# noce2/FluidFramework

Hardware: AMD Instinct MI355X
Metric: sequenced merge-tree ops applied/sec (node) at 100k docs; bit-exact text+props (higher is better)
Workload: dtype int32; 1 GPU; c3: 100000 docs/GPU x 10000 sequenced ops, 8 writers, refSeq lag <= 64, insert 0.5 / remove 0.3 / annotate 0.2; docs_total=100000, docs_per_gpu=100000, ops_per_doc=10000, parallelism=doc-shard x1

## Files before the change

fluidframework_amd/csrc/mt_engine.h:

```cpp
#pragma once
#include <type_traits>

#include "mt_device.h"

#define LDS_AS __attribute__((address_space(3)))
#define GLB_AS __attribute__((address_space(1)))

template <bool kLogT> struct TierLdsT {
    static constexpr bool kLds = true;
    static constexpr bool kLog = kLogT;
    static constexpr bool kPaged = false;
    static constexpr bool kLive = false;
    static constexpr int kOvlBits = 32;
    static constexpr bool kMayGrow = false;
    static constexpr bool kOvf = false;
    typedef uint32_t O_v;
    typedef LDS_AS v4i *A_t;
    typedef LDS_AS uint32_t *O_t;
    typedef LDS_AS v4u *B_t;
    typedef LDS_AS v2i *H_t;
};
template <bool kLogT> struct TierGlbT {
    static constexpr bool kLds = false;
    static constexpr bool kLog = kLogT;
// ... 1980 lines not shown
        const int kept = scour_range(d, bstart, b, 1);
        if (d.status) return;
        wsync<T>();
        if (lane() == 0) d.flg[b] = 0;
        wsync<T>();
        if (kept < old && kept < MT_HALF && d.depth > 1)
            pack(d, 0, b);
        else if (kept < old && ordon(d))
            ord_canon(d, 0, b);
    }
}

TD bool lds_room(DocT<T> &d, const mt_op_rec &op) {
    if (d.n + 3 > d.S_cap) return false;
    if (d.depth + 2 > MT_LV) return false;
    const int nb0 = nbr(d, 0);
    int need_heap = op.kind == MT_OP_INSERT ? 1 : nb0 + 3;
    if (d.heap_n + need_heap > d.H_cap) return false;
    bool ok = true;
    for (int l = 0; l < d.depth; l++) ok = ok && nbr(d, l) + 3 + 24 <= bcap(d, l);
    if (op.kind == MT_OP_REMOVE && oslot_short(d, op_cli(op))) ok = false;
    return ok;
}

TD int live_room(DocT<T> &d, const mt_op_rec &op) {
    if (d.n + 3 > d.S_cap) return 1;
    for (int l = 0; l < d.depth; l++)
        if (nbr(d, l) + 3 + 24 > bcap(d, l)) return 2;
    const int nb0 = nbr(d, 0);
    if (d.heap_n + (op.kind == MT_OP_INSERT ? 1 : nb0 + 3) > d.H_cap) return 3;
    const int nt = op.kind == MT_OP_INSERT && !(op.flags & MT_F_MARKER) ? max(op.pos2, 0) : 0;
    const int tslack = max(d.T_cap / 8, 4096);
    if (d.text_top + nt + tslack > d.T_cap) {
        text_gc(d);
        if (d.text_top + nt + tslack > d.T_cap) return 4;
    }
    const int span = op.kind == MT_OP_ANNOTATE ? min(max(op.pos2 - op.pos1, 0), d.n) + 2 : 0;
    const int np = span + (op.props != MT_NO_PROPS ? 1 : 0) + MT_WAVE;
    if (d.props_top + np > d.P_cap) {
        props_gc(d);
        if (d.props_top + np > d.P_cap) return 5;
    }
    if ((op.flags & MT_F_LOCAL) && d.g_n + 1 > d.LG) return 12;
    return 0;
}

struct OpIn {
    mt_op_rec op;
    u64 pay_lo, pay_hi;
    bool pay_ok;
    bool nl;
    bool pay_lane = false;
    uint32_t pay_v = 0;
};

__device__ __forceinline__ uint16_t pay_unit(const OpIn &in, int j) {
    const u64 w = j < 4 ? (in.pay_lo >> (16 * j)) : (in.pay_hi >> (16 * (j - 4)));
    return (uint16_t)(w & 0xFFFF);
}

TD int first_v0(DocT<T> &d, int from) {
    for (int base = from; base < d.n; base += MT_WAVE) {
        const int i = base + lane();
        const bool v = i < d.n;
        v4i a;
        u64 o;
        load_ao(d, i, v, a, o);
        const u64 m = ballot(v && obs_len(a) > 0);
        if (m) return base + first_lane(m);
    }
    return -1;
}

#ifdef MT_PROF
TD void op_insert_impl(DocT<T> &d, const OpIn &in, const GLB_AS uint16_t *tin, const GLB_AS uint32_t *pin);
TD void op_insert(DocT<T> &d, const OpIn &in, const GLB_AS uint16_t *tin, const GLB_AS uint32_t *pin) {
    PROF_WRAP_BEGIN
    op_insert_impl(d, in, tin, pin);
    PROF_WRAP_END(6)
    
}
TD void op_insert_impl(DocT<T> &d, const OpIn &in, const GLB_AS uint16_t *tin, const GLB_AS uint32_t *pin) {
#else
TD void op_insert(DocT<T> &d, const OpIn &in, const GLB_AS uint16_t *tin, const GLB_AS uint32_t *pin) {
#endif
    const mt_op_rec &op = in.op;
    const int r = op.ref_seq, c = op_cli(op), seq = op.seq, p = op.pos1;
    const bool quiet = (op.flags & MT_F_LOAD) != 0;
    const bool marker = (op.flags & MT_F_MARKER) != 0;
    const int slen = marker ? 1 : op.pos2;
    if (slen > 0 && !marker && !text_ensure(d, slen)) return;
    if (slen > 0 && op.props != MT_NO_PROPS && !props_ensure(d, 1)) return;
    P2_T0(13)
    int carry = 0, split_i = -1, split_q = 0, ip = -1, js = -1;
    for (int base = 0; base < d.n; base += MT_WAVE) {
        const int i = base + lane();
        const bool v = i < d.n;
        v4i a;
        u64 o;
        load_ao(d, i, v, a, o);
        const int vl = v ? vlen(d, a, o, r, c) : 0;
        const int inc = wave_scan_incl(vl);
        const int pex = carry + inc - vl, pin_ = carry + inc;
        const u64 ms = ballot(v && pex < p && p < pin_);
        if (ms) {
            const int l = first_lane(ms);
            split_i = base + l;
// ... 16 lines not shown
        if (ballot(v && pex > p)) break;
    }
    P2_T1(13)
    if (split_i >= 0) {
        split_seg(d, split_i, split_q);
        if (d.status) return;
        ip = js = split_i + 1;
    } else if (ip < 0 && carry == p) {
        ip = d.n;
    }
    Cb cb;
    if (!quiet) cb = cb_begin(d, (T::kLive && d.lop) ? -1 : seq, MT_OP_INSERT);
    if (slen == 0) {
        if (quiet) return;
        cb.n = 1;
        cb_log(d, -1);
        cb_log(d, 0);
        if constexpr (T::kLog) {
            if (d.rich && cb_room(d, 2 + (op.props != MT_NO_PROPS ? 2 * (int)(pin[op.props] & 0xFFFF) : 0))) {
                int np = -1;
                if (op.props != MT_NO_PROPS) {
                    const GLB_AS uint32_t *rec = pin + op.props;
                    np = 0;
                    for (uint32_t j = 0; j < (rec[0] & 0xFFFF); j++) {
                        if (rec[2 + 2 * j] == MT_VAL_NULL) continue;
                        if (lane() == 0) {
                            d.dlog[d.dlog_n + 2 + 2 * np] = (int32_t)rec[1 + 2 * j];
                            d.dlog[d.dlog_n + 3 + 2 * np] = (int32_t)rec[2 + 2 * j];
                        }
                        np++;
                    }
                }
                if (lane() == 0) {
                    d.dlog[d.dlog_n] = (np >= 0 ? 2 : 0) | (ordon(d) ? 4 : 0);
                    d.dlog[d.dlog_n + 1] = np;
                }
                d.dlog_n += 2 + 2 * max(np, 0);
                cb_log_ext(d, 0u, 0, -1, false);
            }
        }
        cb.h = fnv_u64(cb.h, fnv_u32(fnv_u32(MT_FNV_OFF, (uint32_t)-1), 0u));
        cb_end(d, cb);
        return;
    }
    if (ip < 0) {
        fail(d, MT_DOC_INSERT_FAILED);
        return;
    }
    if (d.n + 1 > d.S_cap) {
        fail_cap(d, 1);
        return;
    }
    uint32_t ph = 0, nomatch = 0;
    if (op.props != MT_NO_PROPS) {
        ph = (uint32_t)d.props_top;
        d.props_top++;
        const GLB_AS uint32_t *rec = pin + op.props;
        const uint32_t cntk = rec[0] & 0xFFFF;
        int cn = 0;
        for (uint32_t j = 0; j < cntk; j++) cn += rec[2 + 2 * j] != MT_VAL_NULL;
        if (cn > MT_KMAX) {
            fail(d, MT_DOC_CAPACITY);
            return;
        }
        if (lane() == 0) {
            GLB_AS uint32_t *t = prec(d, d.props_half, ph);
            uint32_t n = 0;
            for (uint32_t j = 0; j < cntk; j++) {
                if (rec[2 + 2 * j] == MT_VAL_NULL) continue;
                t[1 + 2 * n] = rec[1 + 2 * j];
                t[2 + 2 * n] = rec[2 + 2 * j];
                n++;
            }
            t[0] = n;
        }
#ifndef MT_NO_Q4
        bool nm = false;
        for (uint32_t j = 0; j < cntk; j++) {
            const uint32_t v = rec[2 + 2 * j];
            nm = nm || (v != MT_VAL_NULL && (v & MT_VAL_NOMATCH_BIT));
        }
        if (nm) nomatch = SEGF_NOMATCH;
#endif
#ifndef MT_NO_PSIG
        uint32_t sig = 0;
        for (uint32_t j = 0; j < cntk; j++) {
            const uint32_t v = rec[2 + 2 * j];
            if (v != MT_VAL_NULL) sig += mt_psig_mix(rec[1 + 2 * j], v);
        }
        nomatch = psig_put(nomatch, sig);
#endif
    }
    int bstart;
    int B = blk_find(d, 0, ip, false, bstart);
    if (B < 0) {
        FAIL_INTERNAL(d);
        return;
    }
    int bend = bstart + cntr(d, 0, B);
    int x = (js >= 0 && js < bend) ? js : bend;
    if constexpr (T::kLive) {
        while (!d.lop && x == bend) {
            const int s0 = first_v0(d, bend);
            if (s0 < 0 || !is_local_seq(uni(d.A[s0].y)) || B + 1 >= nbr(d, 0)) break;
            B++;
            bstart = bend;
            bend += cntr(d, 0, B);
            x = (js >= 0 && js < bend) ? js : bend;
        }
    }
    uint32_t toff, segw = 0;
    if (marker) {
        toff = op.payload;
    } else {
        toff = (uint32_t)d.text_top;
        GLB_AS uint16_t *dst = text_base(d, d.text_half) + d.text_top;
        bool anynl = false, lastnl = false;
        if (in.pay_ok) {
            const uint16_t u = lane() < slen ? (in.pay_lane ? (uint16_t)in.pay_v : pay_unit(in, lane())) : (uint16_t)0;
            if (lane() < slen) dst[lane()] = u;
            anynl = ballot(lane() < slen && u == (uint16_t)'\n') != 0ull;
            lastnl = ballot(lane() == slen - 1 && u == (uint16_t)'\n') != 0ull;
        } else {
            for (int j = lane(); j < slen; j += MT_WAVE) {
                const uint16_t u = tin[op.payload + j];
                dst[j] = u;
                anynl = anynl || u == (uint16_t)'\n';
                lastnl = lastnl || (j == slen - 1 && u == (uint16_t)'\n');
            }
            anynl = ballot(anynl) != 0ull;
            lastnl = ballot(lastnl) != 0ull;
        }
#ifdef MT_NO_NONL
        anynl = true;
#endif
        d.text_top += slen;
        segw = SEGF_NL_KNOWN | (lastnl ? SEGF_NL : 0u) | (anynl ? 0u : SEGF_NONL);
    }
    P2_T0(15)
    seg_move_right(d, x, 1);
    P2_T1(15)
    mark_dirty(d, x);
    const uint32_t uid = (uint32_t)d.next_uid;
    if (lane() == 0) {
        d.A[x] = v4i{slen, seq, MT_RSEQ_NONE, pack_cli(c, 0)};
// ... 159 lines not shown
            npd++;
        }
        uint32_t nv = v;
#ifndef MT_NO_Q4
        if (comb == MT_COMBINE_TABLE) {
            const GLB_AS uint32_t *tab = rec + 1 + 2 * cntk;
            nv = tab[1];
            if (!absent) {
                const uint32_t old = t[2 + 2 * idx];
                bool hit = false;
                for (uint32_t q = 0; q < tab[0]; q++)
                    if (tab[2 + 2 * q] == old) {
                        nv = tab[3 + 2 * q];
                        hit = true;
                    }
                if (!hit) return false;
            }
        }
#endif
#ifndef MT_NO_PSIG
        if (idx >= 0) sg -= mt_psig_mix(k, t[2 + 2 * idx]);
        if (nv != MT_VAL_NULL) sg += mt_psig_mix(k, nv);
#endif
        if (nv == MT_VAL_NULL) {
            if (idx >= 0) {
                for (uint32_t q = (uint32_t)idx + 1; q < n; q++) {
                    t[2 * q - 1] = t[2 * q + 1];
                    t[2 * q] = t[2 * q + 2];
                }
                n--;
            }
        } else if (idx >= 0) {
            t[2 + 2 * idx] = nv;
        } else {
            if (n >= MT_KMAX) return false;
            t[1 + 2 * n] = k;
            t[2 + 2 * n] = nv;
            n++;
        }
    }
    t[0] = n;
#ifndef MT_NO_PSIG
    if (psig) *psig = sg;
#endif
    sh = fnv_u32(sh, (uint32_t)npd);
    if (nomatch && *nomatch) {
        bool nm = false;
        for (uint32_t q = 0; q < n; q++) nm = nm || (t[2 + 2 * q] & MT_VAL_NOMATCH_BIT) != 0;
        *nomatch = nm;
    }
    return true;
}

TD bool range_mark(DocT<T> &d, const mt_op_rec &op, const GLB_AS uint32_t *rec, int &carry, int &ocarry,
                   Cb &cb) {
    const int r = op.ref_seq, c = op_cli(op), seq = op.seq, p1 = op.pos1, p2 = op.pos2;
    const bool rem = op.kind == MT_OP_REMOVE;
    compute_ends(d);
    if (!rem) gsync_rd();
    int last_b = -1;
    const int L = lane();
    const int nblk = nbr(d, 0);
    bool rec_nm = false;
#ifndef MT_NO_Q4
    if (!rem) {
        rec_nm = (rec[0] >> 16) == MT_COMBINE_TABLE;
        for (uint32_t j = 0; j < (rec[0] & 0xFFFFu); j++) {
            const uint32_t v = rec[2 + 2 * j];
            rec_nm = rec_nm || (v != MT_VAL_NULL && (v & MT_VAL_NOMATCH_BIT));
        }
    }
#endif
    for (int base = 0; base < d.n; base += MT_WAVE) {
        if (!rem && !props_ensure(d, MT_WAVE)) return true;
        const int i = base + L;
        const bool v = i < d.n;
        v4i a;
        u64 o;
        load_ao(d, i, v, a, o);
        const v4u bv = d.Bv[v ? i : 0];
        const int vl = v ? vlen(d, a, o, r, c) : 0;
        const int inc = wave_scan_incl(vl);
        const int pex = carry + inc - vl, pin_ = carry + inc;
        const bool sel = v && vl > 0 && pex < p2 && pin_ > p1;
        const u64 sel_m = ballot(sel);
        if (sel_m) mark_dirty(d, base + first_lane(sel_m));
        bool newly = false, bad = false, spill = false, want_ovf = false;
        bool lrem = false;
        if constexpr (T::kLive) lrem = rem && sel && !d.lop && is_local_seq(a.z);
        const bool ovl_any = rem && ballot(sel && a.z != MT_RSEQ_NONE && !lrem);
        if (ovl_any) {
            if (d.ocs == 0) d.ocs = oslot_take(d, c);
            if (d.ocs > 32) d.wide = 1;
            if (d.ocs && lane() == 0) d.oslot[2 * (d.ocs - 1) + 1] = seq;
        }
        if (rem && sel) {
            if (lrem) {
                a.z = seq;
                a.w = pack_cli(seg_cli(a), c);
                d.A[i] = a;
            } else if (a.z != MT_RSEQ_NONE) {
                bool ovf = false;
                if constexpr (T::kPaged && T::kOvf) ovf = d.ocs == 0 || (o & MT_OVF_BIT);
                if (ovf) {
                    want_ovf = true;
                } else if (d.ocs == 0) {
                    if (T::kOvlBits < 64)
                        spill = true;
                    else
                        bad = true;
                } else {
                    d.O[i] = (typename T::O_v)(o | (1ull << (d.ocs - 1)));
                }
            } else {
                newly = true;
                a.z = seq;
                a.w = pack_cli(seg_cli(a), c);
                d.A[i] = a;
                if constexpr (T::kLive) {
                    if (d.lop) {
                        PendQ pq = pq_get(d, i);
                        if (pq_push(pq, d.lg))
                            pq_put(d, i, pq);
                        else
                            bad = true;
                    }
                }
            }
        }
        if constexpr (T::kPaged && T::kOvf) {
            if (ballot(want_ovf) && !ovf_mark(d, want_ovf, i, o, c, seq)) bad = true;
        }
        uint32_t nh = 0;
        if (!rem && sel) nh = (uint32_t)(d.props_top + __popcll(sel_m & ((1ull << L) - 1ull)));
        const int ol = v ? obs_len(a) : 0;
        const int oinc = wave_scan_incl(ol);
        const int opos = ocarry + oinc - ol;
        const bool entry = rem ? newly : sel;
        u64 sh = fnv_u32(fnv_u32(MT_FNV_OFF, (uint32_t)opos), (uint32_t)a.x);
        if (!rem && sel) {
            int unused = 0;
            bool nm = rec_nm || (bv.w & SEGF_NOMATCH) != 0;
            PendQ pw = pq_zero();
            if constexpr (T::kLive) {
                PendQ pq = pq_get(d, i);
                if (d.lop) {
                    if (pq_push(pq, d.lg))
                        pq_put(d, i, pq);
                    else
                        bad = true;
                } else {
                    pw = pq;
                }
            }
            uint32_t sg = psig_of(bv.w);
            if (!annotate_record(d, bv.y, nh, rec, sh, (GLB_AS int32_t *)nullptr, unused, &nm, pw, nullptr, &sg))
                bad = true;
            v4u nb = bv;
            nb.y = nh;
            nb.w = psig_put((bv.w & ~SEGF_NOMATCH) | (nm ? SEGF_NOMATCH : 0u), sg);
            d.Bv[i] = nb;
        }
        if (ballot(bad)) {
            if (ovl_any && d.ocs == 0 && d.status == 0) d.cap_cause = 11;
            fail(d, MT_DOC_CAPACITY);
            return true;
        }
        if (ballot(spill)) {
            fail_cap(d, 1);
            return true;
        }
        if (!rem) d.props_top += __popcll(sel_m);
        wsync<T>();
        u64 em = ballot(entry);
        while (em) {
            const int j = first_lane(em);
            em &= em - 1;
            cb.h = fnv_u64(cb.h, bcast64(sh, j));
            cb.n++;
            if (T::kLog && d.dlog) {
                cb_log(d, bcast(opos, j));
                cb_log(d, bcast(a.x, j));
                if (!rem) {
                    const uint32_t ohj = (uint32_t)bcast((int)bv.y, j), nhj = (uint32_t)bcast((int)nh, j);
                    int nl = 0;
                    u64 dummy = 0;
                    gsync_rd();
                    if (cb_room(d, 1 + 2 * (MT_KMAX + (int)(rec[0] & 0xFFFF)))) {
                        const int at = d.dlog_n + 1;
                        PendQ pwj = pq_zero();
                        if constexpr (T::kLive) {
                            if (!d.lop) pwj = pq_bcast(pq_get(d, v ? i : 0), j);
                        }
                        if (L == 0) {
                            bool undef = false;
                            annotate_record(d, ohj, nhj, rec, dummy, d.dlog + at, nl, nullptr, pwj, &undef);
                            d.dlog[at - 1] = undef ? -1 : nl / 2;
                        }
                        nl = bcast(nl, 0);
                        d.dlog_n += 1 + nl;
                    }
                }
                if (d.rich) {
                    const v4i aj = v4i{bcast(a.x, j), bcast(a.y, j), bcast(a.z, j), bcast(a.w, j)};
                    v4u bj = v4u{(uint32_t)bcast((int)bv.x, j), (uint32_t)bcast((int)bv.y, j),
                                 (uint32_t)bcast((int)bv.z, j), (uint32_t)bcast((int)bv.w, j)};
                    if (!rem) bj.y = (uint32_t)bcast((int)nh, j);
                    cb_log_seg(d, aj, bj);
                    cb_log_ext(d, bj.z & ~MT_MARKER_BIT, bcast(opos, j), base + j, false);
                }
            }
        }
        const int b = sel ? block_of(d, i, nblk) : -1;
        const u64 below = sel_m & ((1ull << L) - 1ull);
        const int prevl = below ? 63 - __clzll((long long)below) : -1;
// ... 249 lines not shown
```

fluidframework_amd/csrc/mt_kernels.h:

```cpp
#pragma once
#include "../../include/mt_replay.h"
#include "mt_paged.h"

__device__ static void init_doc_hdr(const DevState &st, int doc, int len) {
    DocHdr h;
    memset(&h, 0, sizeof(h));
    h.depth = 1;
    h.n_blk[0] = 1;
    h.text_top = len;
    h.props_top = 1;
    h.next_uid = 2;
    h.delta_hash = MT_FNV_OFF;
    h.status = len > st.T ? MT_DOC_CAPACITY : 0;
    const size_t S = st.S;
    if (len > 0) {
        h.n_seg = 1;
        st.segA[doc * S] = v4i{len, 0, MT_RSEQ_NONE, pack_cli(-1, 0)};
        st.segO[doc * S] = 0ull;
        st.segB[doc * S] = v4u{0u, 0u, 1u, 0u};
        if (st.segP) {
            u64 *w = (u64 *)(st.segP + doc * S);
            w[0] = w[1] = w[2] = w[3] = 0ull;
        }
    }
// ... 517 lines not shown
        if (k < k1) {
            r0 = o4[2 * k];
            r1 = o4[2 * k + 1];
            const int kind = (r1.w >> 16) & 0xFF, flags = ((uint32_t)r1.w >> 24) & 0xFF;
            const int len = r1.x;
#ifdef MT_PAYPF
            if (kind == MT_OP_INSERT && !(flags & MT_F_MARKER) && len > 0) {
                const GLB_AS uint16_t *src = gt + (uint32_t)r1.y;
                if (len <= 8) {
                    pok = 1;
                    uint32_t u[8];
#pragma unroll
                    for (int j = 0; j < 8; j++) u[j] = j < len ? src[j] : 0u;
                    w0 = u[0] | (u[1] << 16);
                    w1 = u[2] | (u[3] << 16);
                    w2 = u[4] | (u[5] << 16);
                    w3 = u[6] | (u[7] << 16);
                }
            }
#endif
        }
        const int cnt = (int)min((int64_t)MT_WAVE, k1 - kb);
        for (int j = 0; j < cnt && w.status == 0; j++) {
            OpIn in;
            in.op.seq = __builtin_amdgcn_readlane(r0.x, j);
            in.op.ref_seq = __builtin_amdgcn_readlane(r0.y, j);
            in.op.min_seq = __builtin_amdgcn_readlane(r0.z, j);
            in.op.pos1 = __builtin_amdgcn_readlane(r0.w, j);
            in.op.pos2 = __builtin_amdgcn_readlane(r1.x, j);
            in.op.payload = (uint32_t)__builtin_amdgcn_readlane(r1.y, j);
            in.op.props = (uint32_t)__builtin_amdgcn_readlane(r1.z, j);
            const uint32_t cw = (uint32_t)__builtin_amdgcn_readlane(r1.w, j);
            in.op.client = (uint16_t)(cw & 0xFFFF);
            in.op.kind = (uint8_t)((cw >> 16) & 0xFF);
            in.op.flags = (uint8_t)(cw >> 24);
            in.pay_lo = (u64)(uint32_t)__builtin_amdgcn_readlane((int)w0, j) |
                        ((u64)(uint32_t)__builtin_amdgcn_readlane((int)w1, j) << 32);
            in.pay_hi = (u64)(uint32_t)__builtin_amdgcn_readlane((int)w2, j) |
                        ((u64)(uint32_t)__builtin_amdgcn_readlane((int)w3, j) << 32);
            in.pay_ok = __builtin_amdgcn_readlane(pok, j) != 0;
            in.nl = false;
            in.pay_lane = false;
            in.pay_v = 0;
#ifndef MT_NO_PAYMSG
            {
                const int len = in.op.pos2;
                if (in.op.kind == MT_OP_INSERT && !(in.op.flags & MT_F_MARKER) && len > 0 && len <= 8) {
                    in.pay_ok = true;
                    in.pay_lane = true;
                    if (lane() < len) in.pay_v = gt[in.op.payload + lane()];
                }
            }
#endif
            if ((pc.tight || pc.grow) && !((pc.grow == 2 || pg_room(pd, in.op)) && pg_arena_room(pd, in.op, pc))) {
                spill_at = kb + j;
                break;
            }
            if (w.status) break;
            pg_apply_op(pd, in, gt, gp);
            pk_ut = max(pk_ut, pd.ut_n);
            pk_heap = max(pk_heap, w.heap_n);
        }
    }
    if (w.status == MT_DOC_RETRY) w.status = MT_DOC_CAPACITY;
    pg_store(pd, st);
    pg_peaks(st, pd, pk_ut, pk_heap);
    if (spill_at >= 0 && w.status == 0)
        pg_handover<T>(st, doc, spill_at, pc);
    else if (k1 < kend && w.status == 0) {
        if (lane() == 0) st.resume[doc] = k1;
    } else if (lane() == 0)
        st.retry[doc] = 0;
#ifdef MT_PROF
    if (st.prof) {
        atomicAdd(&st.prof[lane()], w.prof[lane()]);
        atomicAdd(&st.prof[64 + lane()], w.prof[64 + lane()]);
    }
#endif
}

template <class T>
__global__ void __launch_bounds__(MT_WAVE) k_generate_paged(DevState st, mt_gen_cfg cfg, uint32_t doc_base,
                                                            mt_op_rec *ops_out, uint16_t *text_out,
                                                            uint32_t *props_out, int64_t tstride,
                                                            int64_t pstride, int32_t *fail_out,
                                                            int32_t *dbg_len, int64_t *used_out, PagedCaps pc) {
    extern __shared__ __attribute__((aligned(16))) uint8_t smem_raw[];
    LDS_AS uint8_t *smem = (LDS_AS uint8_t *)smem_raw;
    const int doc = blockIdx.x;
    if (doc >= st.n_docs) return;
    if (st.retry[doc] != pc.stage) return;
    const PagedLayout L = paged_layout(pc.PP, pc.PH, pc.UT, 2 * (cfg.writers + 1), (int)sizeof(typename T::O_v));
    GenCtx g;
    gen_begin(g, st, cfg, (int)(doc_base + doc), doc, smem + L.offGen, tstride, pstride);
    PagedDoc<T> pd;
    pg_setup(pd, st, doc, smem, L, pc);
    DocT<T> &w = pd.w;
    if (w.status || !pg_convert(pd, flat_src(st, doc))) {
        if (lane() == 0) {
            if (pc.tight && w.status == MT_DOC_CAPACITY) {
                st.retry[doc] = 2;
                atomicAdd(st.stats + 12, 1u);
            } else {
                fail_out[doc] = w.status == MT_DOC_RETRY ? MT_DOC_CAPACITY : w.status;
                st.retry[doc] = 0;
            }
// ... 71 lines not shown
```

fluidframework_amd/csrc/mt_paged.h:

```cpp
#pragma once
#include "mt_engine.h"

#ifdef MT_PROF
#define PG_T0(k) const unsigned long long _pt##k = __builtin_amdgcn_s_memtime();
#define PG_T1(k)                                                         \
    if (lane() == 0) {                                                   \
        pd.w.prof[k] += __builtin_amdgcn_s_memtime() - _pt##k;           \
        pd.w.prof[64 + k] += 1ull;                                       \
    }
#define PG_CNT(k)                                                        \
    if (lane() == 0) pd.w.prof[64 + k] += 1ull;
#else
#define PG_T0(k)
#define PG_T1(k)
#define PG_CNT(k)
#endif

template <class T> struct PagedDoc {
    DocT<T> w;
    DocT<T> up;
    LDS_AS PageMeta *meta;
    GLB_AS PageMeta *gmeta;
    LDS_AS int *pvl;
    LDS_AS int *cob;
    LDS_AS int *cdl;
    int vgen, scr_ch;
    LDS_AS uint16_t *upage;
    LDS_AS v4i *uA;
    LDS_AS typename T::O_v *uO;
    LDS_AS uint32_t *uL, *uS, *uP;
    int sbase;
    LDS_AS u64 *uM;
    LDS_AS uint32_t *mbm;
    GLB_AS v4i *gA;
    GLB_AS u64 *gO;
    GLB_AS v4u *gB;
    GLB_AS uint16_t *gumap;
    GLB_AS uint16_t *goS;
    GLB_AS uint16_t *goL;
    int doc;
    int PP, PH, UT, UM;
    int PPh;
    int ut_n;
    int cur;
    int cur_pos;
    int dirty;
    int tdirty;
    int uid_lo;
    int vvalid, vr, vc;
    int zuid, zpv;
    GLB_AS uint16_t *govf;
    int ovf_top, ovf_last, OA;
    int ovf_maxn, ovf_half;
    uint32_t ovf_made;
    int ovf_peak;
    int press;
    int wgrow, opbound;
    LDS_AS int *sob;
    int sob_ch;
    int wnb, wobs;
};

struct PagedCaps {
    int PP, PH, UT;
    int tight;
// ... 1647 lines not shown
            const int lp = uni((int)pd.up.dir[pos]);
            start -= pg_page_view(pd, pos);
            ostart -= uni(pm_obs(pd, lp));
        }
    }
    if (pos < 0) {
        if (slen == 0) {
            if (op.flags & MT_F_LOAD) return;
            Cb cb = cb_begin(w, op.seq, MT_OP_INSERT);
            cb.n = 1;
            cb_log(w, -1);
            cb_log(w, 0);
            cb.h = fnv_u64(cb.h, fnv_u32(fnv_u32(MT_FNV_OFF, (uint32_t)-1), 0u));
            cb_end(w, cb);
            return;
        }
        fail(w, MT_DOC_INSERT_FAILED);
        return;
    }
    pg_load_pos(pd, pos, ostart);
    if (w.status) return;
    OpIn rel = in;
    rel.op.pos1 = op.pos1 - start;
    pd.vvalid = 0;
    pd.tdirty = 1;
    op_insert(w, rel, tin, pin);
    if (w.status) return;
    pg_win_sync(pd);
    if (T::kLog && w.dfr_rec >= 0) pg_log_deferred(pd);
}

TD void pg_boundary(PagedDoc<T> &pd, int p, int r, int c) {
    pg_views_cached(pd, r, c);
    if (pd.w.status) return;
    int start;
    int ostart;
    const int pos = pg_find(pd, p, true, start, ostart);
    if (pos < 0 || start >= p) return;
    pg_load_pos(pd, pos, ostart);
    if (pd.w.status) return;
    pd.tdirty = 1;
    boundary(pd.w, p - start, r, c);
    if (pd.w.status) return;
    pg_win_sync(pd);
}

template <class T> constexpr bool pg_range1() {
#ifdef MT_NO_RANGE1
    return false;
#else
    return !T::kLog && !T::kHM && !T::kLive;
#endif
}
TD void pg_op_range(PagedDoc<T> &pd, const mt_op_rec &op, const GLB_AS uint32_t *pin) {
    DocT<T> &w = pd.w;
    const int r = op.ref_seq, c = op_cli(op), p1 = op.pos1, p2 = op.pos2;
    const bool rem = op.kind == MT_OP_REMOVE;
    const GLB_AS uint32_t *rec = (!rem && op.props != MT_NO_PROPS) ? pin + op.props : nullptr;
    if (rec && (rec[0] >> 16) == MT_COMBINE_OTHER) {
        fail(w, MT_DOC_UNSUPPORTED);
        return;
    }
    if (!rec) rec = (const GLB_AS uint32_t *)&kEmptyPropsRec;
    int step = 0;
    if constexpr (pg_range1<T>()) {
        pg_views_cached(pd, r, c);
        if (w.status) return;
        int start;
        int ostart;
        const int pos = pg_find(pd, p1, true, start, ostart);
        if (pos >= 0 && p1 < p2 && p2 < start + uni(pd.pvl[pos])) {
            if (lane() == 0) pg_zcount(pd)[3]++;
            pg_load_pos(pd, pos, ostart);
            if (w.status) return;
            pd.tdirty = 1;
            const int n0 = w.n;
            if (start < p1) {
                boundary(w, p1 - start, r, c);
                if (w.status) return;
                if (w.pend_split) step = 1;
            }
            if (step == 0) {
                boundary(w, p2 - start, r, c);
                if (w.status) return;
                if (w.pend_split) step = 2;
            }
            if (step == 0) {
                if (w.n != n0 && !rem && w.props_top + MT_WAVE > w.P_cap) {
                    pg_win_sync(pd);
                    if (w.status) return;
                }
                Cb cb = cb_begin(w, op.seq, op.kind);
                pd.vvalid = 0;
                int carry = start, ocarry = ostart;
                PG_T0(45)
                range_mark(w, op, rec, carry, ocarry, cb);
                PG_T1(45)
                if (w.status) return;
                pg_win_sync(pd);
                if (w.status) return;
                cb_end(w, cb);
                return;
            }
            if (lane() == 0) pg_zcount(pd)[4]++;
            pg_win_sync(pd);
            if (w.status) return;
        } else {
            if (lane() == 0) pg_zcount(pd)[5]++;
        }
    } else {
        if (lane() == 0) pg_zcount(pd)[5]++;
    }
    if (step < 1) {
        pg_boundary(pd, p1, r, c);
        if (w.status) return;
    }
    if (step < 2) {
        pg_boundary(pd, p2, r, c);
        if (w.status) return;
    }
    Cb cb = cb_begin(w, op.seq, op.kind);
    pg_views_cached(pd, r, c);
    if (w.status) return;
    pd.vvalid = 0;
    int start;
    int ostart;
    int pos = pg_find(pd, p1, true, start, ostart);
    if (pos >= 0) {
        int carry = start, ocarry = ostart;
        const int np = nbr(pd.up, 1);
        while (pos < np && carry < p2) {
            pg_load_pos(pd, pos, ocarry);
            if (w.status) return;
            pd.tdirty = 1;
            PG_T0(45)
            const bool done = range_mark(w, op, rec, carry, ocarry, cb);
            PG_T1(45)
            if (w.status) return;
            pg_win_sync(pd);
            if (w.status) return;
            if (done) break;
            pos = pg_cur_pos(pd) + 1;
        }
    }
    cb_end(w, cb);
}

TD void pg_renumber(PagedDoc<T> &pd, bool soft = false) {
    DocT<T> &w = pd.w;
    pg_win_flush(pd);
    if (w.status) return;
    pd.cur = -1;
    pd.cur_pos = -1;
    pd.vvalid = 0;
    gsync();
    const int np = nbr(pd.up, 1);
    if (2 * pd.PP > w.T_cap) {
        pg_fail_cap(w, 4);
        return;
    }
    GLB_AS int32_t *first = (GLB_AS int32_t *)text_base(w, 1 - w.text_half);
    int carry = 1;
    for (int base = 0; base < np; base += MT_WAVE) {
        const int q = base + lane();
        const int pg = q < np ? (int)pd.up.dir[q] : 0;
        const int ns = q < np ? pm_nseg(pd, pg) : 0;
        const int inc = wave_scan_incl(ns);
        if (q < np) first[pg] = carry + inc - ns;
        carry += bcast(inc, MT_WAVE - 1);
    }
    gsync();
    gsync_rd();
    const int i = lane();
    for (int e = 1; e <= w.heap_n; e++) {
        const uint32_t uid = (uint32_t)uni(w.heap[e].y);
        int nid = 0;
        if (uid != 0) {
            const int mp = uid < (uint32_t)pd.UM ? uni((int)pd.gumap[uid]) : -1;
            for (int q = (mp >= 0 ? -1 : 0); q < (mp >= 0 ? 0 : np); q++) {
                const int pg = q < 0 ? mp : uni((int)pd.up.dir[q]);
                if (pg >= pd.PP) continue;
                const int ns = uni(pm_nseg(pd, pg));
                const bool hit = i < ns && (pd.gB[(size_t)pg * MT_PG_SLOTS + i].z & ~MT_MARKER_BIT) == uid;
                const u64 m = ballot(hit);
                if (m) {
                    nid = uni((int)first[pg]) + first_lane(m);
                    break;
                }
            }
        }
// ... 62 lines not shown
            FAIL_INTERNAL(w);
            return;
        }
        pg_win_switch(pd, pg);
        if (w.status) return;
        i = find_uid(w, uid);
        if (i < 0) {
            FAIL_INTERNAL(w);
            return;
        }
    }
    pd.tdirty = 1;
    load_removed(w, op);
    if (w.status) return;
    pg_win_sync(pd);
}

TD void pg_apply_op_impl(PagedDoc<T> &pd, const OpIn &in, const GLB_AS uint16_t *tin, const GLB_AS uint32_t *pin) {
    DocT<T> &w = pd.w;
    const mt_op_rec &op = in.op;
    w.ocs = oslot_of(w, op_cli(op));
    if (w.next_uid + 4 > pd.UM && op.kind != MT_OP_LOAD_REMOVED) {
        pg_renumber(pd);
        if (w.status) return;
    }
#ifdef MT_ZPF
    {
        pd.zuid = 0;
        if (w.heap_n > 0 && op.kind != MT_OP_NOOP) {
            const v2i top = heap_top(w);
            if (top.x <= max(w.min_seq, op.min_seq) && top.y > 0 && top.y < pd.UM) {
                pd.zuid = top.y;
                pd.zpv = pd.gumap[top.y];
            }
        }
    }
#endif
    if (op.flags & MT_F_LOAD) {
        const int rich = w.rich;
        w.rich = 0;
        if (op.kind == MT_OP_INSERT)
            pg_op_insert(pd, in, tin, pin);
        else if (op.kind == MT_OP_LOAD_REMOVED)
            pg_load_removed(pd, op);
        else if (op.kind == MT_OP_LOAD_ALIASED)
            fail(w, MT_DOC_ALIASED);
        w.rich = rich;
        return;
    }
    const bool is_op = op.kind == MT_OP_INSERT || op.kind == MT_OP_REMOVE || op.kind == MT_OP_ANNOTATE;
    if (op.kind == MT_OP_INSERT) {
        pg_op_insert(pd, in, tin, pin);
    } else if (is_op) {
        pg_op_range(pd, op, pin);
    }
    if (w.status) return;
    bool z = is_op;
    for (int pass = 0; pass < 2; pass++) {
        if (z) {
            pg_zamboni(pd);
            if (w.status) return;
        }
        if (pass == 1) break;
        if (op.kind != MT_OP_NOOP) {
            if (!(w.cur_seq < op.seq)) {
                fail(w, MT_DOC_SEQ_ORDER);
                return;
            }
            if (!(w.min_seq <= op.min_seq)) {
                fail(w, MT_DOC_MINSEQ_ORDER);
                return;
            }
        }
        z = false;
        if (!(op.flags & MT_F_GROUP_MORE)) {
            if (!(w.cur_seq <= op.seq)) {
                fail(w, MT_DOC_SEQ_BACKWARDS);
                return;
            }
            w.cur_seq = op.seq;
            if (!(op.min_seq <= op.seq)) {
                fail(w, MT_DOC_MSN_ABOVE_SEQ);
                return;
            }
            if (!(w.min_seq <= op.min_seq)) {
                fail(w, MT_DOC_MSN_BACKWARDS);
                return;
            }
            if (op.min_seq > w.min_seq) {
                w.min_seq = op.min_seq;
                z = true;
            }
        }
        if (!z) break;
    }
}

TD void paged_text_compact(DocT<T> &w) {
    PagedDoc<T> &pd = pdoc(w);
    const int keep = pd.cur, keep_pos = pd.cur_pos, keep_td = pd.tdirty;
    if (keep >= 0) pd.dirty = 1;
    pg_win_flush(pd);
    if (w.status) return;
    gsync_rd();
    const int dh = 1 - w.text_half;
    GLB_AS uint16_t *dst = text_base(w, dh);
    const GLB_AS uint16_t *src = text_base(w, w.text_half);
// ... 796 lines not shown
```

Baseline: 176.3 million ops/s.

## Lane-parallelize property record parsing and add per-lane annotate fast path

The record header word is prefetched into a lane register when ops are staged, so it is no longer re-read from global memory. Insert-time property copying becomes wave-parallel: each lane reads one record word, compacts non-null entries with a ballot and rank, and writes them out. Annotate gains an annotate_lanes fast path that keeps the props record in lane registers and merges small existing property sets (up to MT_ANN1_B entries) per lane instead of calling the serial annotate_record. It also adds MT_PROF timing hooks, and the new merge logic has to reproduce the hash and signature semantics bit-exactly.

After: 177.5 million ops/s (median of 6 runs). Within noise of the previous version (+0.7%).

```diff
diff --git a/fluidframework_amd/csrc/mt_engine.h b/fluidframework_amd/csrc/mt_engine.h
--- a/fluidframework_amd/csrc/mt_engine.h
+++ b/fluidframework_amd/csrc/mt_engine.h
@@ -2056,7 +2056,15 @@
     bool nl;
     bool pay_lane = false;
     uint32_t pay_v = 0;
+    bool rec_lane = false;
 };
+#define MT_REC0_LANE 8
+__device__ __forceinline__ uint32_t rec_word0(const OpIn &in, const GLB_AS uint32_t *rec) {
+#ifndef MT_NO_PROPLANE
+    if (in.rec_lane) return (uint32_t)__builtin_amdgcn_readlane((int)in.pay_v, MT_REC0_LANE);
+#endif
+    return (uint32_t)uni((int)rec[0]);
+}
 
 __device__ __forceinline__ uint16_t pay_unit(const OpIn &in, int j) {
     const u64 w = j < 4 ? (in.pay_lo >> (16 * j)) : (in.pay_hi >> (16 * (j - 4)));
@@ -2179,45 +2187,89 @@
         return;
     }
     uint32_t ph = 0, nomatch = 0;
+#ifdef MT_PROF
+    const unsigned long long _tp = __builtin_amdgcn_s_memtime();
+#endif
     if (op.props != MT_NO_PROPS) {
         ph = (uint32_t)d.props_top;
         d.props_top++;
         const GLB_AS uint32_t *rec = pin + op.props;
+#ifndef MT_NO_PROPLANE
+        const uint32_t cntk = rec_word0(in, rec) & 0xFFFF;
+        if (T::kPaged && cntk < MT_WAVE / 2) {
+            const int L = lane();
+            const uint32_t rv = L < 1 + 2 * (int)cntk ? rec[L] : 0u;
+            const uint32_t rk = (uint32_t)__shfl((int)rv, L > 0 ? L - 1 : 0, MT_WAVE);
+            const bool nn = L >= 2 && !(L & 1) && L <= 2 * (int)cntk && rv != MT_VAL_NULL;
+            const u64 m = ballot(nn);
+            const int cn = __popcll(m);
+            if (cn > MT_KMAX) {
+                fail(d, MT_DOC_CAPACITY);
+                return;
+            }
+            GLB_AS uint32_t *t = prec(d, d.props_half, ph);
+            if (nn) {
+                const int rank = __popcll(m & ((1ull << L) - 1ull));
+                t[1 + 2 * rank] = rk;
+                t[2 + 2 * rank] = rv;
+            }
+            if (L == 0) t[0] = (uint32_t)cn;
+#ifndef MT_NO_Q4
+            if (ballot(nn && (rv & MT_VAL_NOMATCH_BIT))) nomatch = SEGF_NOMATCH;
+#endif
+#ifndef MT_NO_PSIG
+            nomatch = psig_put(nomatch, (uint32_t)wave_sum((int)(nn ? mt_psig_mix(rk, rv) : 0u)));
+#endif
+        } else {
+#else
         const uint32_t cntk = rec[0] & 0xFFFF;
-        int cn = 0;
-        for (uint32_t j = 0; j < cntk; j++) cn += rec[2 + 2 * j] != MT_VAL_NULL;
-        if (cn > MT_KMAX) {
-            fail(d, MT_DOC_CAPACITY);
-            return;
-        }
+        {
+#endif
+            int cn = 0;
+            for (uint32_t j = 0; j < cntk; j++) cn += rec[2 + 2 * j] != MT_VAL_NULL;
+            if (cn > MT_KMAX) {
+                fail(d, MT_DOC_CAPACITY);
+                return;
+            }
+            if (lane() == 0) {
+                GLB_AS uint32_t *t = prec(d, d.props_half, ph);
+                uint32_t n = 0;
+                for (uint32_t j = 0; j < cntk; j++) {
+                    if (rec[2 + 2 * j] == MT_VAL_NULL) continue;
+                    t[1 + 2 * n] = rec[1 + 2 * j];
+                    t[2 + 2 * n] = rec[2 + 2 * j];
+                    n++;
+                }
+                t[0] = n;
+            }
+#ifndef MT_NO_Q4
+            bool nm = false;
+            for (uint32_t j = 0; j < cntk; j++) {
+                const uint32_t v = rec[2 + 2 * j];
+                nm = nm || (v != MT_VAL_NULL && (v & MT_VAL_NOMATCH_BIT));
+            }
+            if (nm) nomatch = SEGF_NOMATCH;
+#endif
+#ifndef MT_NO_PSIG
+            uint32_t sig = 0;
+            for (uint32_t j = 0; j < cntk; j++) {
+                const uint32_t v = rec[2 + 2 * j];
+                if (v != MT_VAL_NULL) sig += mt_psig_mix(rec[1 + 2 * j], v);
+            }
+            nomatch = psig_put(nomatch, sig);
+#endif
+    }
+    }
+#ifdef MT_PROF
+    if (op.props != MT_NO_PROPS) {
+        uint32_t nmv = nomatch;
+        asm volatile("" : "+v"(nmv));
         if (lane() == 0) {
-            GLB_AS uint32_t *t = prec(d, d.props_half, ph);
-            uint32_t n = 0;
-            for (uint32_t j = 0; j < cntk; j++) {
-                if (rec[2 + 2 * j] == MT_VAL_NULL) continue;
-                t[1 + 2 * n] = rec[1 + 2 * j];
-                t[2 + 2 * n] = rec[2 + 2 * j];
-                n++;
-            }
-            t[0] = n;
-        }
-#ifndef MT_NO_Q4
-        bool nm = false;
-        for (uint32_t j = 0; j < cntk; j++) {
-            const uint32_t v = rec[2 + 2 * j];
-            nm = nm || (v != MT_VAL_NULL && (v & MT_VAL_NOMATCH_BIT));
-        }
-        if (nm) nomatch = SEGF_NOMATCH;
-#endif
-#ifndef MT_NO_PSIG
-        uint32_t sig = 0;
-        for (uint32_t j = 0; j < cntk; j++) {
-            const uint32_t v = rec[2 + 2 * j];
-            if (v != MT_VAL_NULL) sig += mt_psig_mix(rec[1 + 2 * j], v);
-        }
-        nomatch = psig_put(nomatch, sig);
-#endif
-    }
+            d.prof[50] += __builtin_amdgcn_s_memtime() - _tp;
+            d.prof[64 + 50] += 1ull;
+        }
+    }
+#endif
     int bstart;
     int B = blk_find(d, 0, ip, false, bstart);
     if (B < 0) {
@@ -2483,8 +2535,134 @@
     return true;
 }
 
+#ifndef MT_NO_ANN1
+#ifndef MT_ANN1_B
+#define MT_ANN1_B 4
+#endif
+TD bool annotate_lanes(DocT<T> &d, bool want, uint32_t oh, uint32_t nh, uint32_t rv, int cntk, bool rw,
+                       u64 &sh_io, bool &nm_io, uint32_t &sg_io, bool &ovf) {
+    constexpr int B = MT_ANN1_B;
+    uint32_t ok[B], ov[B];
+    uint32_t on = 0;
+#pragma unroll
+    for (int i = 0; i < B; i++) ok[i] = ov[i] = 0;
+    if (want && oh) {
+        const GLB_AS uint32_t *o = prec(d, d.props_half, oh);
+        on = o[0];
+#pragma unroll
+        for (int i = 0; i < B; i++) {
+            ok[i] = o[1 + 2 * i];
+            ov[i] = o[2 + 2 * i];
+        }
+    }
+    const bool fast = want && on <= (uint32_t)B;
+    if (!ballot(fast)) return false;
+    uint32_t alive = fast ? (1u << on) - 1u : 0u;
+    uint32_t delrw = 0;
+    uint32_t app = 0;
+    u64 sh = sh_io;
+    uint32_t sg = sg_io;
+    int npd = 0;
+    if (rw) {
+#pragma unroll
+        for (int i = 0; i < B; i++) {
+            bool in_new = false, truthy = false;
+            for (int j = 0; j < cntk; j++) {
+                const uint32_t kj = (uint32_t)bcast((int)rv, 1 + 2 * j), vj = (uint32_t)bcast((int)rv, 2 + 2 * j);
+                if (ok[i] == kj) {
+                    in_new = true;
+                    truthy = vj != MT_VAL_NULL && !(vj & MT_VAL_FALSY_BIT);
+                }
+            }
+            if (((alive >> i) & 1u) && !truthy) {
+                sh = fnv_u32(fnv_u32(sh, ok[i]), in_new ? MT_VAL_NULL : ov[i]);
+                npd++;
+#ifndef MT_NO_PSIG
+                sg -= mt_psig_mix(ok[i], ov[i]);
+#endif
+                alive &= ~(1u << i);
+                delrw |= 1u << i;
+            }
+        }
+    }
+    int n = __popc(alive);
+    for (int j = 0; j < cntk; j++) {
+        const uint32_t kj = (uint32_t)bcast((int)rv, 1 + 2 * j), vj = (uint32_t)bcast((int)rv, 2 + 2 * j);
+        uint32_t hit = 0, cur = 0;
+        bool dbr = false;
+#pragma unroll
+        for (int i = 0; i < B; i++) {
+            if (ok[i] == kj) {
+                if ((alive >> i) & 1u) {
+                    hit = 1u << i;
+                    cur = ov[i];
+                }
+                dbr = dbr || ((delrw >> i) & 1u);
+            }
+        }
+        if (fast && !ovf) {
+            if (!(dbr && !hit)) {
+                sh = fnv_u32(fnv_u32(sh, kj), (!hit || cur == MT_VAL_UNDEF) ? MT_VAL_NULL : cur);
+                npd++;
+            }
+#ifndef MT_NO_PSIG
+            if (hit) sg -= mt_psig_mix(kj, cur);
+            if (vj != MT_VAL_NULL) sg += mt_psig_mix(kj, vj);
+#endif
+            if (vj == MT_VAL_NULL) {
+                if (hit) {
+                    alive &= ~hit;
+                    n--;
+                }
+            } else if (hit) {
+#pragma unroll
+                for (int i = 0; i < B; i++)
+                    if ((hit >> i) & 1u) ov[i] = vj;
+            } else if (n >= MT_KMAX) {
+                ovf = true;
+            } else {
+                app |= 1u << j;
+                n++;
+            }
+        }
+    }
+    const bool st = fast && !ovf;
+    GLB_AS uint32_t *t = prec(d, d.props_half, st ? nh : 0u);
+    bool nm = false;
+    int pos = 0;
+    if (st) {
+#pragma unroll
+        for (int i = 0; i < B; i++) {
+            if ((alive >> i) & 1u) {
+                t[1 + 2 * pos] = ok[i];
+                t[2 + 2 * pos] = ov[i];
+                nm = nm || (ov[i] & MT_VAL_NOMATCH_BIT) != 0;
+                pos++;
+            }
+        }
+        t[0] = (uint32_t)n;
+        sh_io = fnv_u32(sh, (uint32_t)npd);
+        sg_io = sg;
+    }
+    if (ballot(app != 0)) {
+        for (int j = 0; j < cntk; j++) {
+            const uint32_t kj = (uint32_t)bcast((int)rv, 1 + 2 * j), vj = (uint32_t)bcast((int)rv, 2 + 2 * j);
+            if (st && ((app >> j) & 1u)) {
+                t[1 + 2 * pos] = kj;
+                t[2 + 2 * pos] = vj;
+                nm = nm || (vj & MT_VAL_NOMATCH_BIT) != 0;
+                pos++;
+            }
+        }
+    }
+    if (st && nm_io) nm_io = nm;
+    return fast;
+}
+#endif
+
+#define MT_REC0_NONE 0xFFFFFFFFu
 TD bool range_mark(DocT<T> &d, const mt_op_rec &op, const GLB_AS uint32_t *rec, int &carry, int &ocarry,
-                   Cb &cb) {
+                   Cb &cb, uint32_t w0_in = MT_REC0_NONE) {
     const int r = op.ref_seq, c = op_cli(op), seq = op.seq, p1 = op.pos1, p2 = op.pos2;
     const bool rem = op.kind == MT_OP_REMOVE;
     compute_ends(d);
@@ -2493,6 +2671,39 @@
     const int L = lane();
     const int nblk = nbr(d, 0);
     bool rec_nm = false;
+#ifndef MT_NO_ANN1
+    uint32_t rv = 0;
+    int rl_cntk = 0;
+    bool rl_ok = false, rl_rw = false;
+    if (!rem) {
+        const uint32_t w0 = w0_in != MT_REC0_NONE ? w0_in : (uint32_t)uni((int)rec[0]);
+        const uint32_t cntk = w0 & 0xFFFFu, comb = w0 >> 16;
+        if (cntk <= MT_KMAX) {
+            if (L < 1 + 2 * (int)cntk) rv = rec[L];
+            const bool isval = L >= 2 && L <= 2 * (int)cntk && !(L & 1);
+#ifndef MT_NO_Q4
+            rec_nm = comb == MT_COMBINE_TABLE ||
+                     ballot(isval && rv != MT_VAL_NULL && (rv & MT_VAL_NOMATCH_BIT)) != 0;
+#endif
+            bool dup = false;
+            for (int j = 0; j < (int)cntk; j++) {
+                const uint32_t kj = (uint32_t)bcast((int)rv, 1 + 2 * j);
+                dup = dup || __popcll(ballot((L & 1) && L < 1 + 2 * (int)cntk && rv == kj)) > 1;
+            }
+            rl_cntk = (int)cntk;
+            rl_rw = comb == MT_COMBINE_REWRITE;
+            rl_ok = !dup && (comb == MT_COMBINE_NONE || rl_rw);
+        } else {
+#ifndef MT_NO_Q4
+            rec_nm = comb == MT_COMBINE_TABLE;
+            for (uint32_t j = 0; j < cntk; j++) {
+                const uint32_t v = rec[2 + 2 * j];
+                rec_nm = rec_nm || (v != MT_VAL_NULL && (v & MT_VAL_NOMATCH_BIT));
+            }
+#endif
+        }
+    }
+#else
 #ifndef MT_NO_Q4
     if (!rem) {
         rec_nm = (rec[0] >> 16) == MT_COMBINE_TABLE;
@@ -2501,6 +2712,7 @@
             rec_nm = rec_nm || (v != MT_VAL_NULL && (v & MT_VAL_NOMATCH_BIT));
         }
     }
+#endif
 #endif
     for (int base = 0; base < d.n; base += MT_WAVE) {
         if (!rem && !props_ensure(d, MT_WAVE)) return true;
@@ -2569,11 +2781,22 @@
         const int opos = ocarry + oinc - ol;
         const bool entry = rem ? newly : sel;
         u64 sh = fnv_u32(fnv_u32(MT_FNV_OFF, (uint32_t)opos), (uint32_t)a.x);
-        if (!rem && sel) {
-            int unused = 0;
-            bool nm = rec_nm || (bv.w & SEGF_NOMATCH) != 0;
-            PendQ pw = pq_zero();
-            if constexpr (T::kLive) {
+#ifdef MT_PROF
+        const unsigned long long _ta = __builtin_amdgcn_s_memtime();
+        if (!rem && sel_m) {
+            const uint32_t onp = (sel && bv.y) ? prec(d, d.props_half, bv.y)[0] : 0u;
+            for (uint32_t q = 0; q <= MT_KMAX; q++) {
+                const int c = __popcll(ballot(sel && onp == q));
+                if (lane() == 0) d.prof[64 + 51 + q] += (u64)c;
+            }
+        }
+        const unsigned long long _tb = __builtin_amdgcn_s_memtime();
+#endif
+        bool nm = rec_nm || (bv.w & SEGF_NOMATCH) != 0;
+        PendQ pw = pq_zero();
+        uint32_t sg = psig_of(bv.w);
+        if constexpr (T::kLive) {
+            if (!rem && sel) {
                 PendQ pq = pq_get(d, i);
                 if (d.lop) {
                     if (pq_push(pq, d.lg))
@@ -2584,14 +2807,38 @@
                     pw = pq;
                 }
             }
-            uint32_t sg = psig_of(bv.w);
-            if (!annotate_record(d, bv.y, nh, rec, sh, (GLB_AS int32_t *)nullptr, unused, &nm, pw, nullptr, &sg))
+        }
+        bool served = false;
+#ifndef MT_NO_ANN1
+        if (rl_ok) {
+            const bool want = sel && !(T::kLive && pq_any(pw));
+            if (ballot(want)) {
+                bool ovf = false;
+                served = annotate_lanes(d, want, bv.y, nh, rv, rl_cntk, rl_rw, sh, nm, sg, ovf);
+                if (ovf) bad = true;
+            }
+        }
+#endif
+        if (!rem && sel) {
+            int unused = 0;
+            if (!served &&
+                !annotate_record(d, bv.y, nh, rec, sh, (GLB_AS int32_t *)nullptr, unused, &nm, pw, nullptr, &sg))
                 bad = true;
             v4u nb = bv;
             nb.y = nh;
             nb.w = psig_put((bv.w & ~SEGF_NOMATCH) | (nm ? SEGF_NOMATCH : 0u), sg);
             d.Bv[i] = nb;
         }
+#ifdef MT_PROF
+        if (!rem && sel_m) {
+            gsync_rd();
+            if (lane() == 0) {
+                d.prof[48] += __builtin_amdgcn_s_memtime() - _tb;
+                d.prof[64 + 48] += 1ull;
+            }
+        }
+        (void)_ta;
+#endif
         if (ballot(bad)) {
             if (ovl_any && d.ocs == 0 && d.status == 0) d.cap_cause = 11;
             fail(d, MT_DOC_CAPACITY);
diff --git a/fluidframework_amd/csrc/mt_kernels.h b/fluidframework_amd/csrc/mt_kernels.h
--- a/fluidframework_amd/csrc/mt_kernels.h
+++ b/fluidframework_amd/csrc/mt_kernels.h
@@ -593,6 +593,12 @@
                 }
             }
 #endif
+#ifndef MT_NO_PROPLANE
+            if (in.op.props != MT_NO_PROPS && (in.op.kind == MT_OP_INSERT || in.op.kind == MT_OP_ANNOTATE)) {
+                in.rec_lane = true;
+                if (lane() == MT_REC0_LANE) in.pay_v = gp[in.op.props];
+            }
+#endif
             if ((pc.tight || pc.grow) && !((pc.grow == 2 || pg_room(pd, in.op)) && pg_arena_room(pd, in.op, pc))) {
                 spill_at = kb + j;
                 break;
diff --git a/fluidframework_amd/csrc/mt_paged.h b/fluidframework_amd/csrc/mt_paged.h
--- a/fluidframework_amd/csrc/mt_paged.h
+++ b/fluidframework_amd/csrc/mt_paged.h
@@ -10,7 +10,13 @@
     }
 #define PG_CNT(k)                                                        \
     if (lane() == 0) pd.w.prof[64 + k] += 1ull;
+#define PG_T1K(k, s)                                                     \
+    if (lane() == 0) {                                                   \
+        pd.w.prof[s] += __builtin_amdgcn_s_memtime() - _pt##k;           \
+        pd.w.prof[64 + (s)] += 1ull;                                     \
+    }
 #else
+#define PG_T1K(k, s)
 #define PG_T0(k)
 #define PG_T1(k)
 #define PG_CNT(k)
@@ -1764,12 +1770,27 @@
     return !T::kLog && !T::kHM && !T::kLive;
 #endif
 }
-TD void pg_op_range(PagedDoc<T> &pd, const mt_op_rec &op, const GLB_AS uint32_t *pin) {
+TD void pg_op_range(PagedDoc<T> &pd, const OpIn &in, const GLB_AS uint32_t *pin) {
     DocT<T> &w = pd.w;
+    const mt_op_rec &op = in.op;
     const int r = op.ref_seq, c = op_cli(op), p1 = op.pos1, p2 = op.pos2;
     const bool rem = op.kind == MT_OP_REMOVE;
     const GLB_AS uint32_t *rec = (!rem && op.props != MT_NO_PROPS) ? pin + op.props : nullptr;
-    if (rec && (rec[0] >> 16) == MT_COMBINE_OTHER) {
+    PG_T0(49)
+    const uint32_t w0 = rec ? rec_word0(in, rec) : 0u;
+#ifdef MT_PROF
+    if (rec) {
+        uint32_t wv = w0;
+        asm volatile("" : "+v"(wv));
+        PG_T1(49)
+        if (lane() == 0) {
+            const uint32_t ck = w0 & 0xFFFFu;
+            pd.w.prof[64 + (ck <= 1 ? 60 : ck == 2 ? 61 : 62)] += 1ull;
+            if ((w0 >> 16) == MT_COMBINE_TABLE) pd.w.prof[64 + 63] += 1ull;
+        }
+    }
+#endif
+    if ((w0 >> 16) == MT_COMBINE_OTHER) {
         fail(w, MT_DOC_UNSUPPORTED);
         return;
     }
@@ -1806,8 +1827,9 @@
                 pd.vvalid = 0;
                 int carry = start, ocarry = ostart;
                 PG_T0(45)
-                range_mark(w, op, rec, carry, ocarry, cb);
+                range_mark(w, op, rec, carry, ocarry, cb, w0);
                 PG_T1(45)
+                PG_T1K(45, rem ? 47 : 46)
                 if (w.status) return;
                 pg_win_sync(pd);
                 if (w.status) return;
@@ -1846,8 +1868,9 @@
             if (w.status) return;
             pd.tdirty = 1;
             PG_T0(45)
-            const bool done = range_mark(w, op, rec, carry, ocarry, cb);
+            const bool done = range_mark(w, op, rec, carry, ocarry, cb, w0);
             PG_T1(45)
+            PG_T1K(45, rem ? 47 : 46)
             if (w.status) return;
             pg_win_sync(pd);
             if (w.status) return;
@@ -2016,7 +2039,7 @@
     if (op.kind == MT_OP_INSERT) {
         pg_op_insert(pd, in, tin, pin);
     } else if (is_op) {
-        pg_op_range(pd, op, pin);
+        pg_op_range(pd, in, pin);
     }
     if (w.status) return;
     bool z = is_op;
```
